# MahdiGhafoorian/NLML_HPE

Hardware: AMD Instinct MI355X
Metric: faces_per_sec (higher is better)
Workload: dtype f16x2s

## Files before the change

nlml_hpe_amd/csrc/encoder_heads_f16x2_w8.hip:

```cpp
#include <hip/hip_runtime.h>

#include "../../include/nlml_hpe.h"
#include "abi_internal.h"
#include "encoder_heads_f16x2_dev.h"
#include "layout.h"

#if defined(W8_TAIL_EXIT) && defined(__HIP_DEVICE_COMPILE__) && !defined(__gfx950__) && !defined(__gfx942__)
#error "-DW8_TAIL_EXIT relies on S_BARRIER ignoring terminated waves (gfx942 / gfx950)"
#endif

namespace nlml {
namespace hx {

__device__ __forceinline__ double div_ipd_w8(double n, double d, double y) {
  const double q = n * y;
  const double r = fma(-q, d, n);
  return fma(r, y, q);
}

template <typename XHi, typename XLo, typename Extra>
__device__ __forceinline__ void step_w8(f32x16 (&acc)[2][2], f32x16 (&accS)[2][2], const h8 (&wcur)[2][2], const h8 (&xh)[2], h8 (&xl)[2],
                                        h8 (&wnext_hi)[2][2], const h8* __restrict__ wp_hi, h8 (&wnext_lo)[2][2], const h8* __restrict__ wp_lo,
                                        XHi xload_hi, XLo xload_lo, Extra extra) {
#pragma unroll
  for (int m = 0; m < 12; ++m) {
    const int t = m / 4, nb = (m % 4) / 2, fb = m % 2;
    if (t == 0) accS[nb][fb] = __builtin_amdgcn_mfma_f32_32x32x16_f16(wcur[nb][1], xh[fb], accS[nb][fb], 0, 0, 0);
    else if (t == 1) accS[nb][fb] = __builtin_amdgcn_mfma_f32_32x32x16_f16(wcur[nb][0], xl[fb], accS[nb][fb], 0, 0, 0);
    else acc[nb][fb] = __builtin_amdgcn_mfma_f32_32x32x16_f16(wcur[nb][0], xh[fb], acc[nb][fb], 0, 0, 0);
    __builtin_amdgcn_sched_barrier(0);
    if (m == 0) xload_hi(0);
    if (m == 1) xload_hi(1);
    if (m == 2) wnext_hi[0][0] = wp_hi[0];
    if (m == 4) wnext_lo[0][1] = wp_lo[64];
    if (m == 6) wnext_hi[1][0] = wp_hi[128];
    if (m == 8) xload_lo(0);
    if (m == 9) xload_lo(1);
    if (m == 10) wnext_lo[1][1] = wp_lo[192];
    extra(m);
    __builtin_amdgcn_sched_barrier(0);
  }
}

template <bool VEC4, bool NORM>
__device__ __forceinline__ void stage_e0_pass_w8(const Ctx& c, const Args& a, int64_t row0, int tid, int pass, int jw, int nbh,
                                                 f32x16 (&acc)[2][2], f32x16 (&accS)[2][2]) {
  constexpr int NB = 2, NFB = 2;
  constexpr int WSTEP = 4 * 2 * 64;
  const int F = a.F;
  const int nslab = (int)c.hdr.k8_e0 / XS_STEPS;

  const int srow = tid >> 3, scol = (tid & 7) * 4;
  int64_t r = row0 + srow;
  const bool live = r < a.B;
  r = live ? r : a.B - 1;
  const float* p = a.x + r * a.ldx;
  double ipd = 1.0, rcp = 1.0, ra = 0.0, rb = 0.0, rc = 0.0;
  if (NORM) {
    const double dx = (double)p[99] - (double)p[789], dy = (double)p[100] - (double)p[790], dz = (double)p[101] - (double)p[791];
    ipd = sqrt(fma(dz, dz, fma(dy, dy, dx * dx)));
    if (ipd == 0.0) ipd = 1e-6;
    rcp = 1.0 / ipd;
    const double x0 = (double)p[3], y0 = (double)p[4], z0 = (double)p[5];
    const int ph = scol % 3;
    ra = ph == 0 ? x0 : (ph == 1 ? y0 : z0);
    rb = ph == 0 ? y0 : (ph == 1 ? z0 : x0);
    rc = ph == 0 ? z0 : (ph == 1 ? x0 : y0);
  }
  unsigned nzbits = 0u;

#ifndef W8_XLINE
  const bool adv = false;
#else
  const int xphase = (int)((reinterpret_cast<uintptr_t>(p) >> 4) & 7);
  const bool adv = VEC4 && xphase != 0 && xphase + (tid & 7) < 8;
#endif

  struct Set { float v[4]; };
  [[maybe_unused]] Set carry;
  auto gload_at = [&](int s, Set& st) {
    s = s < nslab ? s : nslab - 1;
#ifdef W8_ABL_XHOT
    s = 0;
#endif
    const int k = s * XS_COLS + scol;
    if (VEC4) {
      const int kc = k < F ? k : (NORM ? k - 12 * ((k - F + 15) / 12) : F - 4);
#ifdef W8_X_NT
      const f32x4 t = __builtin_nontemporal_load(reinterpret_cast<const f32x4*>(p + kc));
#else
      const f32x4 t = *reinterpret_cast<const f32x4*>(p + kc);
#endif
#pragma unroll
      for (int e = 0; e < 4; ++e) st.v[e] = t[e];
    } else {
#pragma unroll
      for (int e = 0; e < 4; ++e) st.v[e] = p[k + e < F ? k + e : F - 1];
    }
  };
  auto gload = [&](int s, Set& st) { gload_at(s + (adv ? 1 : 0), st); };
  auto lw_begin = [&](Set& st) {
#pragma unroll
    for (int e = 0; e < 4; ++e) asm volatile("" : "+v"(st.v[e]));
#ifdef W8_XLINE
    if (VEC4) {
#pragma unroll
      for (int e = 0; e < 4; ++e) {
        const float t = st.v[e];
        st.v[e] = adv ? carry.v[e] : t;
        carry.v[e] = t;
      }
    }
#endif
  };
  auto lw_norm = [&](Set& st, int q) {
    const int t = q % 3;
    const double rr = t == 0 ? ra : (t == 1 ? rb : rc);
    st.v[q] = (float)div_ipd_w8((double)st.v[q] - rr, ipd, rcp);
  };
  auto lw_rotate = [&]() {
    const double t0 = rc; rc = rb; rb = ra; ra = t0;
  };
  typedef unsigned u2 __attribute__((ext_vector_type(2)));
  unsigned pend_hi[2], pend_lo[2];
  auto lw_split = [&](Set& st, int j, bool real_slab) {
    const unsigned m = real_slab ? 0x7fffffffu : 0u;
    nzbits |= (__float_as_uint(st.v[2 * j]) | __float_as_uint(st.v[2 * j + 1])) & m;
    split2(st.v[2 * j], st.v[2 * j + 1], pend_hi[j], pend_lo[j]);
  };
  constexpr int XW_PLANE = 64 * 64, XW_SLAB = 2 * XW_PLANE, XW_BUF = 2 * XW_SLAB, O_XW = LDS_BYTES - 2 * XW_BUF;
  static_assert(O_XW >= 16 * 512 * 16, "slabs behind the parked accumulators");
  const int wr_off = srow * 64 + ((((tid & 7) >> 1) ^ ((srow >> 2) & 3)) << 4) + 8 * (tid & 1);
  auto lw_store = [&](int slab_off, int piece) {
    char* d = c.lds + O_XW + slab_off + wr_off;
    if (piece == 0) *reinterpret_cast<u2*>(d) = u2{pend_hi[0], pend_hi[1]};
    else *reinterpret_cast<u2*>(d + XW_PLANE) = u2{pend_lo[0], pend_lo[1]};
  };
  auto lwrite = [&](int slab_off, Set& st, bool real_slab) {
    lw_begin(st);
    if (NORM) {
#pragma unroll
      for (int q = 0; q < 4; ++q) lw_norm(st, q);
      lw_rotate();
    }
#pragma unroll
    for (int j = 0; j < 2; ++j) lw_split(st, j, real_slab);
    lw_store(slab_off, 0);
    lw_store(slab_off, 1);
  };

  const int job = 4 * pass + jw;
  load_bias<NB, NFB>(acc, c.blob4 + c.hdr.b_off(ST_E0) + job * (4 * 8) + (2 * nbh) * 8, c.h);
  zero_acc<NB, NFB>(accS);
  const h8* w = c.blob8 + c.hdr.w_off(ST_E0) + (size_t)job * c.hdr.job_w16(ST_E0) + (2 * nbh * 2) * 64 + c.lane;
#ifdef W8_ABL_WHOT
  auto wfrag = [&](int ks) { return w + (size_t)(ks & 3) * WSTEP; };
#elif defined(W8_ABL_WL2)
  auto wfrag = [&](int ks) { return w + (size_t)((ks & 3) + 4 * (blockIdx.x % 20)) * WSTEP; };
#else
  auto wfrag = [&](int ks) { return w + (size_t)ks * WSTEP; };
#endif

  Set set[2];
#ifndef W8_D0_HI
#define W8_D0_HI 2
#endif
#ifndef W8_D0_LO
#define W8_D0_LO 2
#endif
  constexpr int R0 = 4, DH = W8_D0_HI, DL = W8_D0_LO;
  h8 wr[R0][NB][2];
#ifdef W8_XLINE
  if (VEC4) gload_at(0, carry);
#endif
  gload(0, set[0]);
  gload(1, set[1]);
  lwrite(0, set[0], true);
  lwrite(XW_SLAB, set[1], true);
  gload(2, set[0]);
  gload(3, set[1]);
#pragma unroll
  for (int d = 0; d < (DH > DL ? DH : DL); ++d)
#pragma unroll
    for (int nb = 0; nb < NB; ++nb)
#pragma unroll
      for (int pp = 0; pp < 2; ++pp)
        if (d < (pp ? DL : DH)) wr[d][nb][pp] = wfrag(d)[(nb * 2 + pp) * 64];
  __syncthreads();

  const int rd0 = c.f * 64 + ((c.h ^ ((c.f >> 2) & 3)) << 4);
  typedef __attribute__((address_space(3))) const char LdsC;
  LdsC* const xb0 = (LdsC*)(c.lds + O_XW + rd0);
  LdsC* const xb1 = (LdsC*)(c.lds + O_XW + (rd0 ^ 32));
  h8 xh[2][NFB], xl[NFB];
  auto xread = [&](LdsC* base, int t, int fb, int pp) {
    return *reinterpret_cast<const __attribute__((address_space(3))) h8*>(base + (t >> 1) * XW_SLAB + pp * XW_PLANE + fb * (32 * 64));
  };
  const int niter = nslab / 2;
#pragma unroll
  for (int fb = 0; fb < NFB; ++fb) {
    xh[0][fb] = xread(xb0, 0, fb, 0);
    xl[fb] = xread(xb0, 0, fb, 1);
  }
#ifdef W8_XTOUCH
  unsigned xt_sink = 0;
  auto xtouch = [&](int k, int slab0) {
    int64_t rr = row0 + 8 * c.wv + (k & 7);
    rr = rr < a.B ? rr : a.B - 1;
    int col = (slab0 + (k >> 3)) * XS_COLS + XS_COLS - 1;
    col = col < F ? col : F - 1;
    const float* q = a.x + rr * a.ldx + col;
    asm volatile("s_load_dword %0, %1, 0x0" : "+s"(xt_sink) : "s"(q) : "memory");
  };
#endif
  int cur = 0, nxt = XW_BUF;
  for (int it = 0; it < niter; ++it) {
    const int s = 2 * it;
    LdsC* xc[2] = {xb0 + cur, xb1 + cur};
    LdsC* xn = xb0 + nxt;
    asm volatile("" : "+v"(xc[0]), "+v"(xc[1]), "+v"(xn));
#pragma unroll
    for (int t = 0; t < 4; ++t) {
      const int ks = 4 * it + t;
#ifndef W8_ABL_NOBAR
      if (t == 3) __syncthreads();
#endif
#ifdef W8_XTOUCH
      if (t == 3) asm volatile("s_waitcnt lgkmcnt(0)" : "+s"(xt_sink));
#endif
      step_w8(acc, accS, wr[t], xh[t & 1], xl, wr[(t + DH) % R0], wfrag(ks + DH), wr[(t + DL) % R0], wfrag(ks + DL),
              [&](int fb) { xh[(t + 1) & 1][fb] = t < 3 ? xread(xc[(t + 1) & 1], t + 1, fb, 0) : xread(xn, 0, fb, 0); },
              [&](int fb) { xl[fb] = t < 3 ? xread(xc[(t + 1) & 1], t + 1, fb, 1) : xread(xn, 0, fb, 1); },
              [&](int m) {
#ifdef W8_ABL_NOSTAGE
                return;
#endif
#ifdef W8_XTOUCH
                if (t == 3) {
                  if (m < 4) { xtouch(2 * m, s + 6); xtouch(2 * m + 1, s + 6); }
                  else xtouch(4 + m, s + 6);
                }
#endif
                if (t >= 2) return;
                Set& st = set[t & 1];
                const int j = m;
                const bool real = s + t + 2 < nslab;
                if (j == 0) lw_begin(st);
                if (NORM && j >= 1 && j < 5) lw_norm(st, j - 1);
                if (NORM && j == 5) lw_rotate();
                if (j == 6 || j == 7) lw_split(st, j - 6, real);
                if (j == 8) lw_store(nxt + t * XW_SLAB, 0);
                if (j == 9) lw_store(nxt + t * XW_SLAB, 1);
                if (j == 11) gload(s + t + 4, st);
              });
    }
    const int t0 = cur; cur = nxt; nxt = t0;
  }
#ifdef W8_XTOUCH
  asm volatile("s_waitcnt lgkmcnt(0)" : "+s"(xt_sink));
#endif
  if (pass == 0 && a.valid) {
    const unsigned long long m = __ballot(nzbits != 0u);
    if ((tid & 7) == 0 && live) a.valid[row0 + srow] = ((m >> (c.lane & 56)) & 0xFFull) ? 1 : 0;
  }
}

#ifdef HX_STAMPS
#define W8S(i)                                                                                                          \
  do {                                                                                                                  \
    if (a.latent && c.lane == 0)                                                                                        \
      reinterpret_cast<unsigned long long*>(a.latent)[((size_t)blockIdx.x * 8 + c.wv) * 16 + (i)] = __builtin_amdgcn_s_memtime(); \
  } while (0)
#define W8S_WALL(i)                                                                                                     \
  do {                                                                                                                  \
    if (a.latent && c.lane == 0)                                                                                        \
      reinterpret_cast<unsigned long long*>(a.latent)[((size_t)blockIdx.x * 8 + c.wv) * 16 + (i)] = wall_clock64();     \
  } while (0)
#else
#define W8S(i) do { } while (0)
#define W8S_WALL(i) do { } while (0)
#endif

template <bool VEC4, bool NORM, bool TRUNK = false>
__global__ __launch_bounds__(512) void encoder_heads_f16x2_w8_kernel(Args a) {
  __shared__ __attribute__((aligned(16))) char lds[LDS_BYTES];

  const int tid = threadIdx.x;
  Ctx c;
  c.blob8 = reinterpret_cast<const h8*>(a.blob);
  c.blob4 = reinterpret_cast<const f32x4*>(a.blob);
  c.hdr = load_hdr(reinterpret_cast<const Header*>(a.blob));
  c.lds = lds;
  c.lane = tid & 63;
  c.f = c.lane & 31;
  c.h = c.lane >> 5;
  c.wv = __builtin_amdgcn_readfirstlane(tid >> 6);
  const int jw = c.wv >> 1, nbh = c.wv & 1;
  const int64_t row0 = (int64_t)blockIdx.x * TILE_FACES;

  {
    constexpr int WSTEP1 = 4 * 2 * 64;
    const h8* w1 = c.blob8 + c.hdr.w_off(ST_E1) + (size_t)jw * c.hdr.job_w16(ST_E1) + (2 * nbh * 2) * 64 + c.lane;
    const float inv0 = c.hdr.inv_scale[ST_E0];
    f32x16 acc1[2][2];
    f32x4* const park = reinterpret_cast<f32x4*>(c.lds + O_H1H) + tid;
    static_assert(16 * 512 * 16 <= 2 * P_H1H, "the parked layer-1 accumulators fit the h1 half image");
    load_bias<2, 2>(acc1, c.blob4 + c.hdr.b_off(ST_E1) + jw * (4 * 8) + (2 * nbh) * 8, c.h);
    auto park_acc1 = [&]() {
#pragma unroll
      for (int nb = 0; nb < 2; ++nb)
#pragma unroll
        for (int fb = 0; fb < 2; ++fb)
#pragma unroll
          for (int q = 0; q < 4; ++q)
            park[512 * ((nb * 2 + fb) * 4 + q)] = f32x4{acc1[nb][fb][4 * q], acc1[nb][fb][4 * q + 1], acc1[nb][fb][4 * q + 2], acc1[nb][fb][4 * q + 3]};
    };
    park_acc1();
    W8S(0);
    W8S_WALL(14);
#pragma unroll 1
    for (int pass = 0; pass < 2; ++pass) {
      {
        f32x16 acc0[2][2], acc0s[2][2];
        stage_e0_pass_w8<VEC4, NORM>(c, a, row0, tid, pass, jw, nbh, acc0, acc0s);
        add_acc<2, 2>(acc0, acc0s);
        W8S(1 + 4 * pass);
#pragma unroll
        for (int nb = 0; nb < 2; ++nb)
#pragma unroll
          for (int fb = 0; fb < 2; ++fb)
#pragma unroll
            for (int q = 0; q < 4; ++q) {
              const f32x4 t = park[512 * ((nb * 2 + fb) * 4 + q)];
              acc1[nb][fb][4 * q] = t[0]; acc1[nb][fb][4 * q + 1] = t[1]; acc1[nb][fb][4 * q + 2] = t[2]; acc1[nb][fb][4 * q + 3] = t[3];
            }
        __syncthreads();
        job_store<2, 2, ACT_RELU>(c, acc0, O_H1H, P_H1H, S_H1H, 128 * jw + 64 * nbh, 0, inv0);
      }
      __syncthreads();
      W8S(2 + 4 * pass);
      {
        f32x16 acc1s[2][2];
        zero_acc<2, 2>(acc1s);
        kloop<2, 2, 32, WSTEP1>(acc1, acc1s, w1 + (size_t)pass * 32 * WSTEP1, c.lds + O_H1H + (c.f * S_H1H + 8 * c.h) * 2, P_H1H,
                                32 * S_H1H * 2);
        add_acc<2, 2>(acc1, acc1s);
      }
      W8S(3 + 4 * pass);
      __syncthreads();
      if (pass == 0) park_acc1();
      W8S(4 + 4 * pass);
    }
    job_store<2, 2, ACT_RELU>(c, acc1, O_H2, P_H2, S_H2, 128 * jw + 64 * nbh, 0, c.hdr.inv_scale[ST_E1]);
  }
  __syncthreads();
  W8S(9);
  Ctx ct = c;
  ct.wv = c.wv & 3;
  f32x16 acc3[1][2];
  h8 wr3[ring_slots(1, 2)][1][2];
  {
    constexpr int WSTEP2 = 2 * 2 * 64;
    f32x16 acc2[1][2], acc2s[1][2];
    load_bias<1, 2>(acc2, c.blob4 + c.hdr.b_off(ST_E2) + jw * (2 * 8) + nbh * 8, c.h);
    zero_acc<1, 2>(acc2s);
    const h8* w2 = c.blob8 + c.hdr.w_off(ST_E2) + (size_t)jw * c.hdr.job_w16(ST_E2) + (nbh * 2) * 64 + c.lane;
    kloop<1, 2, 32, WSTEP2>(acc2, acc2s, w2, c.lds + O_H2 + (c.f * S_H2 + 8 * c.h) * 2, P_H2, 32 * S_H2 * 2);
    add_acc<1, 2>(acc2, acc2s);
    W8S(10);
    if constexpr (TRUNK) {
      typedef unsigned u4_ __attribute__((ext_vector_type(4)));
      u4_* const dst = reinterpret_cast<u4_*>(a.h3ws) + (size_t)blockIdx.x * (2 * 16 * 2 * 64) + c.lane;
#pragma unroll
      for (int fb = 0; fb < 2; ++fb) {
        h8 fr[2][2];
        frags_from_acc<ACT_RELU>(acc2[0][fb], c.hdr.inv_scale[ST_E2], fr);
#pragma unroll
        for (int p = 0; p < 2; ++p)
#pragma unroll
          for (int pc = 0; pc < 2; ++pc)
            dst[((fb * 16 + 4 * jw + 2 * nbh + p) * 2 + pc) * 64] = __builtin_bit_cast(u4_, fr[p][pc]);
      }
      return;
    }
    tail_pre_e3<false>(ct, acc3, wr3);
    __syncthreads();
    job_store<1, 2, ACT_RELU>(c, acc2, O_H3, P_H3, S_H3, 64 * jw + 32 * nbh, 0, c.hdr.inv_scale[ST_E2]);
  }
  __syncthreads();
  W8S(11);
  W8S_WALL(15);
#ifdef W8_TAIL_EXIT
  if (c.wv >= 4) return;
  constexpr bool H1W8 = false;
#else
  ct.helper = c.wv >= 4 ? 1 : 0;
  constexpr bool H1W8 = true;
#endif
#ifdef HX_STAMPS
  Args at = a;
  if (a.latent) at.latent = a.latent + (size_t)gridDim.x * 8 * 16 * 2;
  tail_stages<false, STRICT_INKERNEL_RESCUE_MAX, H1W8>(ct, at, row0, acc3, wr3);
#else
  tail_stages<false, STRICT_INKERNEL_RESCUE_MAX, H1W8>(ct, a, row0, acc3, wr3);
#endif
}

}

size_t tailws_workspace_bytes(int64_t B, int F) {
  if (B <= 0 || F <= 0) return 0;
  return (size_t)((B + TILE_FACES - 1) / TILE_FACES) * (2 * 16 * 2 * 1024);
}

int launch_encoder_heads_f16x2_tailws(const float* x, int64_t ldx, const float* raw, int normalize, int64_t B, int F,
                                      const void* blob, float* out, float* latent, uint8_t* valid, void* workspace,
                                      size_t ws_bytes, void* stream) {
  if (B == 0) return 0;
  if (!workspace || ws_bytes < tailws_workspace_bytes(B, F)) return fail(NLML_E_BADARG, "streamed-tail path: workspace too small");
  if (reinterpret_cast<uintptr_t>(workspace) & 15) return fail(NLML_E_BADARG, "streamed-tail path: workspace must be 16-byte aligned");
  hx::Args a;
  a.B = B; a.F = F; a.blob = blob; a.out = out; a.latent = latent; a.valid = valid; a.h3ws = workspace;
  const K2Input in = k2_input(x, ldx, raw, normalize, F);
  a.x = in.src; a.ldx = in.ld; a.norm = in.norm;
  if (!in.vec4) return fail(NLML_E_BADARG, "streamed-tail path: x must be 16-byte aligned with F and ldx multiples of 4");
  const int64_t ntiles = (B + TILE_FACES - 1) / TILE_FACES;
  const dim3 grid((unsigned)ntiles), block(512);
  hipStream_t st = reinterpret_cast<hipStream_t>(stream);
  if (a.norm) hipLaunchKernelGGL((hx::encoder_heads_f16x2_w8_kernel<true, true, true>), grid, block, 0, st, a);
  else hipLaunchKernelGGL((hx::encoder_heads_f16x2_w8_kernel<true, false, true>), grid, block, 0, st, a);
  if (int rc = hip_launch_status()) return rc;
  if (int rc = launch_tail_ws(blob, workspace, 2 * ntiles, B, out, latent, stream)) return rc;
  return launch_strict_reeval(x, ldx, raw, normalize, B, F, blob, out, latent, stream);
}

int launch_encoder_heads_f16x2_w8(const float* x, int64_t ldx, const float* raw, int normalize, int64_t B, int F,
                                  const void* blob, float* out, float* latent, uint8_t* valid, void* stream) {
  if (B == 0) return 0;
  hx::Args a;
  a.B = B; a.F = F; a.blob = blob; a.out = out; a.latent = latent; a.valid = valid;
  const K2Input in = k2_input(x, ldx, raw, normalize, F);
  a.x = in.src; a.ldx = in.ld; a.norm = in.norm;
  const dim3 grid((unsigned)((B + TILE_FACES - 1) / TILE_FACES)), block(512);
  hipStream_t st = reinterpret_cast<hipStream_t>(stream);
  k2_with_variant(in, [&](auto V, auto N) {
    hipLaunchKernelGGL((hx::encoder_heads_f16x2_w8_kernel<decltype(V)::value, decltype(N)::value>), grid, block, 0, st, a);
  });
  if (int rc = hip_launch_status()) return rc;
  return launch_strict_reeval(x, ldx, raw, normalize, B, F, blob, out, latent, stream);
}

}
```

Baseline: 79.20 million.

## Reorder layer-0 MFMA/LDS schedule, enable XLINE, deepen weight prefetch, cut register pressure

The layer-0 step now issues the hi*hi MFMAs first and loads the next x-hi fragments late, so the double-buffered xh array becomes a single buffer. The block barrier moves inside the step at m==1 instead of before it. The cache-line-aligned x load path (W8_XLINE) is now on by default, and the weight prefetch distance grows from 2 to 3. Register pressure is also reduced: reference coordinates are kept as floats, address and lane values are recomputed through asm barriers so they are not held across the pass, and the w1 pointer is built later. The intent is to lower VGPR use and improve overlap. The risk is changed latency hiding and the extra prefetch registers.

```diff
diff --git a/nlml_hpe_amd/csrc/encoder_heads_f16x2_w8.hip b/nlml_hpe_amd/csrc/encoder_heads_f16x2_w8.hip
--- a/nlml_hpe_amd/csrc/encoder_heads_f16x2_w8.hip
+++ b/nlml_hpe_amd/csrc/encoder_heads_f16x2_w8.hip
@@ -9,6 +9,16 @@
 #error "-DW8_TAIL_EXIT relies on S_BARRIER ignoring terminated waves (gfx942 / gfx950)"
 #endif
 
+#ifndef W8_XLINE
+#define W8_XLINE 1
+#endif
+#ifndef W8_D0_HI
+#define W8_D0_HI 3
+#endif
+#ifndef W8_D0_LO
+#define W8_D0_LO 3
+#endif
+
 namespace nlml {
 namespace hx {
 
@@ -19,23 +29,23 @@
 }
 
 template <typename XHi, typename XLo, typename Extra>
-__device__ __forceinline__ void step_w8(f32x16 (&acc)[2][2], f32x16 (&accS)[2][2], const h8 (&wcur)[2][2], const h8 (&xh)[2], h8 (&xl)[2],
+__device__ __forceinline__ void step_w8(f32x16 (&acc)[2][2], f32x16 (&accS)[2][2], const h8 (&wcur)[2][2], h8 (&xh)[2], h8 (&xl)[2],
                                         h8 (&wnext_hi)[2][2], const h8* __restrict__ wp_hi, h8 (&wnext_lo)[2][2], const h8* __restrict__ wp_lo,
                                         XHi xload_hi, XLo xload_lo, Extra extra) {
 #pragma unroll
   for (int m = 0; m < 12; ++m) {
     const int t = m / 4, nb = (m % 4) / 2, fb = m % 2;
-    if (t == 0) accS[nb][fb] = __builtin_amdgcn_mfma_f32_32x32x16_f16(wcur[nb][1], xh[fb], accS[nb][fb], 0, 0, 0);
-    else if (t == 1) accS[nb][fb] = __builtin_amdgcn_mfma_f32_32x32x16_f16(wcur[nb][0], xl[fb], accS[nb][fb], 0, 0, 0);
-    else acc[nb][fb] = __builtin_amdgcn_mfma_f32_32x32x16_f16(wcur[nb][0], xh[fb], acc[nb][fb], 0, 0, 0);
+    if (t == 0) acc[nb][fb] = __builtin_amdgcn_mfma_f32_32x32x16_f16(wcur[nb][0], xh[fb], acc[nb][fb], 0, 0, 0);
+    else if (t == 1) accS[nb][fb] = __builtin_amdgcn_mfma_f32_32x32x16_f16(wcur[nb][1], xh[fb], accS[nb][fb], 0, 0, 0);
+    else accS[nb][fb] = __builtin_amdgcn_mfma_f32_32x32x16_f16(wcur[nb][0], xl[fb], accS[nb][fb], 0, 0, 0);
     __builtin_amdgcn_sched_barrier(0);
-    if (m == 0) xload_hi(0);
-    if (m == 1) xload_hi(1);
+    if (m == 0) xload_lo(0);
+    if (m == 1) xload_lo(1);
     if (m == 2) wnext_hi[0][0] = wp_hi[0];
     if (m == 4) wnext_lo[0][1] = wp_lo[64];
     if (m == 6) wnext_hi[1][0] = wp_hi[128];
-    if (m == 8) xload_lo(0);
-    if (m == 9) xload_lo(1);
+    if (m == 8) xload_hi(0);
+    if (m == 9) xload_hi(1);
     if (m == 10) wnext_lo[1][1] = wp_lo[192];
     extra(m);
     __builtin_amdgcn_sched_barrier(0);
@@ -51,17 +61,18 @@
   const int nslab = (int)c.hdr.k8_e0 / XS_STEPS;
 
   const int srow = tid >> 3, scol = (tid & 7) * 4;
-  int64_t r = row0 + srow;
-  const bool live = r < a.B;
-  r = live ? r : a.B - 1;
-  const float* p = a.x + r * a.ldx;
-  double ipd = 1.0, rcp = 1.0, ra = 0.0, rb = 0.0, rc = 0.0;
+  const int64_t left = a.B - 1 - row0;
+  const int last = left < TILE_FACES - 1 ? (int)left : TILE_FACES - 1;
+  const bool live = srow <= last;
+  const float* p = a.x + (row0 + (live ? srow : last)) * a.ldx;
+  double ipd = 1.0, rcp = 1.0;
+  float ra = 0.f, rb = 0.f, rc = 0.f;
   if (NORM) {
     const double dx = (double)p[99] - (double)p[789], dy = (double)p[100] - (double)p[790], dz = (double)p[101] - (double)p[791];
     ipd = sqrt(fma(dz, dz, fma(dy, dy, dx * dx)));
     if (ipd == 0.0) ipd = 1e-6;
     rcp = 1.0 / ipd;
-    const double x0 = (double)p[3], y0 = (double)p[4], z0 = (double)p[5];
+    const float x0 = p[3], y0 = p[4], z0 = p[5];
     const int ph = scol % 3;
     ra = ph == 0 ? x0 : (ph == 1 ? y0 : z0);
     rb = ph == 0 ? y0 : (ph == 1 ? z0 : x0);
@@ -69,7 +80,7 @@
   }
   unsigned nzbits = 0u;
 
-#ifndef W8_XLINE
+#if !W8_XLINE
   const bool adv = false;
 #else
   const int xphase = (int)((reinterpret_cast<uintptr_t>(p) >> 4) & 7);
@@ -102,7 +113,7 @@
   auto lw_begin = [&](Set& st) {
 #pragma unroll
     for (int e = 0; e < 4; ++e) asm volatile("" : "+v"(st.v[e]));
-#ifdef W8_XLINE
+#if W8_XLINE
     if (VEC4) {
 #pragma unroll
       for (int e = 0; e < 4; ++e) {
@@ -115,11 +126,11 @@
   };
   auto lw_norm = [&](Set& st, int q) {
     const int t = q % 3;
-    const double rr = t == 0 ? ra : (t == 1 ? rb : rc);
-    st.v[q] = (float)div_ipd_w8((double)st.v[q] - rr, ipd, rcp);
+    const float rr = t == 0 ? ra : (t == 1 ? rb : rc);
+    st.v[q] = (float)div_ipd_w8((double)st.v[q] - (double)rr, ipd, rcp);
   };
   auto lw_rotate = [&]() {
-    const double t0 = rc; rc = rb; rb = ra; ra = t0;
+    const float t0 = rc; rc = rb; rb = ra; ra = t0;
   };
   typedef unsigned u2 __attribute__((ext_vector_type(2)));
   unsigned pend_hi[2], pend_lo[2];
@@ -162,15 +173,9 @@
 #endif
 
   Set set[2];
-#ifndef W8_D0_HI
-#define W8_D0_HI 2
-#endif
-#ifndef W8_D0_LO
-#define W8_D0_LO 2
-#endif
   constexpr int R0 = 4, DH = W8_D0_HI, DL = W8_D0_LO;
   h8 wr[R0][NB][2];
-#ifdef W8_XLINE
+#if W8_XLINE
   if (VEC4) gload_at(0, carry);
 #endif
   gload(0, set[0]);
@@ -192,16 +197,13 @@
   typedef __attribute__((address_space(3))) const char LdsC;
   LdsC* const xb0 = (LdsC*)(c.lds + O_XW + rd0);
   LdsC* const xb1 = (LdsC*)(c.lds + O_XW + (rd0 ^ 32));
-  h8 xh[2][NFB], xl[NFB];
+  h8 xh[NFB], xl[NFB];
   auto xread = [&](LdsC* base, int t, int fb, int pp) {
     return *reinterpret_cast<const __attribute__((address_space(3))) h8*>(base + (t >> 1) * XW_SLAB + pp * XW_PLANE + fb * (32 * 64));
   };
   const int niter = nslab / 2;
 #pragma unroll
-  for (int fb = 0; fb < NFB; ++fb) {
-    xh[0][fb] = xread(xb0, 0, fb, 0);
-    xl[fb] = xread(xb0, 0, fb, 1);
-  }
+  for (int fb = 0; fb < NFB; ++fb) xh[fb] = xread(xb0, 0, fb, 0);
 #ifdef W8_XTOUCH
   unsigned xt_sink = 0;
   auto xtouch = [&](int k, int slab0) {
@@ -222,23 +224,21 @@
 #pragma unroll
     for (int t = 0; t < 4; ++t) {
       const int ks = 4 * it + t;
+      step_w8(acc, accS, wr[t], xh, xl, wr[(t + DH) % R0], wfrag(ks + DH), wr[(t + DL) % R0], wfrag(ks + DL),
+              [&](int fb) { xh[fb] = t < 3 ? xread(xc[(t + 1) & 1], t + 1, fb, 0) : xread(xn, 0, fb, 0); },
+              [&](int fb) { xl[fb] = xread(xc[t & 1], t, fb, 1); },
+              [&](int m) {
 #ifndef W8_ABL_NOBAR
-      if (t == 3) __syncthreads();
-#endif
-#ifdef W8_XTOUCH
-      if (t == 3) asm volatile("s_waitcnt lgkmcnt(0)" : "+s"(xt_sink));
-#endif
-      step_w8(acc, accS, wr[t], xh[t & 1], xl, wr[(t + DH) % R0], wfrag(ks + DH), wr[(t + DL) % R0], wfrag(ks + DL),
-              [&](int fb) { xh[(t + 1) & 1][fb] = t < 3 ? xread(xc[(t + 1) & 1], t + 1, fb, 0) : xread(xn, 0, fb, 0); },
-              [&](int fb) { xl[fb] = t < 3 ? xread(xc[(t + 1) & 1], t + 1, fb, 1) : xread(xn, 0, fb, 1); },
-              [&](int m) {
+                if (t == 3 && m == 1) __syncthreads();
+#endif
 #ifdef W8_ABL_NOSTAGE
                 return;
 #endif
 #ifdef W8_XTOUCH
                 if (t == 3) {
-                  if (m < 4) { xtouch(2 * m, s + 6); xtouch(2 * m + 1, s + 6); }
-                  else xtouch(4 + m, s + 6);
+                  if (m == 1) asm volatile("s_waitcnt lgkmcnt(0)" : "+s"(xt_sink));
+                  else if (m >= 2 && m < 8) { xtouch(2 * m - 4, s + 6); xtouch(2 * m - 3, s + 6); }
+                  else if (m >= 8) xtouch(4 + m, s + 6);
                 }
 #endif
                 if (t >= 2) return;
@@ -300,13 +300,18 @@
 
   {
     constexpr int WSTEP1 = 4 * 2 * 64;
-    const h8* w1 = c.blob8 + c.hdr.w_off(ST_E1) + (size_t)jw * c.hdr.job_w16(ST_E1) + (2 * nbh * 2) * 64 + c.lane;
     const float inv0 = c.hdr.inv_scale[ST_E0];
     f32x16 acc1[2][2];
-    f32x4* const park = reinterpret_cast<f32x4*>(c.lds + O_H1H) + tid;
     static_assert(16 * 512 * 16 <= 2 * P_H1H, "the parked layer-1 accumulators fit the h1 half image");
     load_bias<2, 2>(acc1, c.blob4 + c.hdr.b_off(ST_E1) + jw * (4 * 8) + (2 * nbh) * 8, c.h);
-    auto park_acc1 = [&]() {
+    auto fresh = [&](Ctx& k) {
+      int t = tid;
+      asm volatile("" : "+v"(t));
+      k.lane = t & 63; k.f = k.lane & 31; k.h = k.lane >> 5;
+      return t;
+    };
+    auto park_acc1 = [&](int t) {
+      f32x4* const park = reinterpret_cast<f32x4*>(c.lds + O_H1H) + t;
 #pragma unroll
       for (int nb = 0; nb < 2; ++nb)
 #pragma unroll
@@ -315,16 +320,20 @@
           for (int q = 0; q < 4; ++q)
             park[512 * ((nb * 2 + fb) * 4 + q)] = f32x4{acc1[nb][fb][4 * q], acc1[nb][fb][4 * q + 1], acc1[nb][fb][4 * q + 2], acc1[nb][fb][4 * q + 3]};
     };
-    park_acc1();
+    park_acc1(tid);
     W8S(0);
     W8S_WALL(14);
 #pragma unroll 1
     for (int pass = 0; pass < 2; ++pass) {
       {
         f32x16 acc0[2][2], acc0s[2][2];
-        stage_e0_pass_w8<VEC4, NORM>(c, a, row0, tid, pass, jw, nbh, acc0, acc0s);
+        Ctx cp = c;
+        const int tp = fresh(cp);
+        stage_e0_pass_w8<VEC4, NORM>(cp, a, row0, tp, pass, jw, nbh, acc0, acc0s);
         add_acc<2, 2>(acc0, acc0s);
         W8S(1 + 4 * pass);
+        const int tq = fresh(c);
+        f32x4* const park = reinterpret_cast<f32x4*>(c.lds + O_H1H) + tq;
 #pragma unroll
         for (int nb = 0; nb < 2; ++nb)
 #pragma unroll
@@ -342,13 +351,14 @@
       {
         f32x16 acc1s[2][2];
         zero_acc<2, 2>(acc1s);
+        const h8* w1 = c.blob8 + c.hdr.w_off(ST_E1) + (size_t)jw * c.hdr.job_w16(ST_E1) + (2 * nbh * 2) * 64 + c.lane;
         kloop<2, 2, 32, WSTEP1>(acc1, acc1s, w1 + (size_t)pass * 32 * WSTEP1, c.lds + O_H1H + (c.f * S_H1H + 8 * c.h) * 2, P_H1H,
                                 32 * S_H1H * 2);
         add_acc<2, 2>(acc1, acc1s);
       }
       W8S(3 + 4 * pass);
       __syncthreads();
-      if (pass == 0) park_acc1();
+      if (pass == 0) park_acc1(fresh(c));
       W8S(4 + 4 * pass);
     }
     job_store<2, 2, ACT_RELU>(c, acc1, O_H2, P_H2, S_H2, 128 * jw + 64 * nbh, 0, c.hdr.inv_scale[ST_E1]);
```

Result: no change. 78.96 million (-0.3%).
